# vsergeev/luaradio

Measured on AMD Instinct MI355X. Metric: MSamples/s per block (128-tap complex FIR headline) + WBFM chain end-to-end, higher is better.
Workload: dtype f32

## Files before the change

luaradio_amd/csrc/kernels_channelizer.h:

```cpp
#pragma once
#include "common.h"
#include "kernels_fir.h"

#ifndef LRHIP_CHAN_EXP
#define LRHIP_CHAN_EXP 0
#endif

namespace lrhip {

#ifndef LRHIP_CHAN_INTERLEAVE
#define LRHIP_CHAN_INTERLEAVE 1
#endif
#ifndef LRHIP_CHAN_RT
#define LRHIP_CHAN_RT 1
#endif
#ifndef LRHIP_CHAN_KSLAB
#define LRHIP_CHAN_KSLAB 32
#endif
constexpr int CHAN_RT = LRHIP_CHAN_RT;
constexpr int CHAN_MT = 64 * CHAN_RT;
constexpr int CHAN_KSLAB = LRHIP_CHAN_KSLAB;

template <int NCT>
__global__ __launch_bounds__(256, CHAN_RT == 1 ? 2 : 1) void channelizer_kernel(const float *__restrict__ hist, const float *__restrict__ x,
                                                             const float *__restrict__ W, float *__restrict__ y,
                                                             int M, long n, long nframes, long first)
{
    constexpr int K2 = 16 * NCT;
    constexpr int K = K2 / 2;
    constexpr int DROW = K2 + 2;
    constexpr int WROW = K2 + 16;
    extern __shared__ __attribute__((aligned(16))) float lds[];
    const int tid = threadIdx.x, lane = tid & 63, wave = tid >> 6;
    const int col = lane & 15, kq = lane >> 4;
    const long f0 = (long)blockIdx.x * CHAN_MT;
    const int nsamp = (CHAN_MT - 1) * K + M;
    const int nflt = 2 * nsamp;
    float *ldsD = lds;
    const int dsize = ((nflt + 2 * (nflt / K2) + 2 + 3) / 4) * 4;
    float *ldsW = lds + dsize;

    const long p0 = first + f0 * K;
    const long xlo = p0 - (M - 1);
    if (xlo >= 0 && xlo + nsamp <= n && ((reinterpret_cast<uintptr_t>(x + 2 * xlo) & 15) == 0)) {
        const float4 *src = reinterpret_cast<const float4 *>(x + 2 * xlo);
        for (int i4 = tid; i4 < nflt / 4; i4 += 256) {
            float4 v = src[i4];
            int a = 4 * i4, p = a + 2 * (a / K2);
            *reinterpret_cast<float2 *>(ldsD + p) = make_float2(v.x, v.y);
            *reinterpret_cast<float2 *>(ldsD + p + 2) = make_float2(v.z, v.w);
        }
        for (int a = (nflt / 4) * 4 + tid; a < nflt; a += 256) ldsD[a + 2 * (a / K2)] = x[2 * xlo + a];
    } else {
        for (int r = tid; r < nsamp; r += 256) {
            int a = 2 * r, p = a + 2 * (a / K2);
            ldsD[p] = stream_at<2>(hist, x, p0 + r, 0, M, n);
            ldsD[p + 1] = stream_at<2>(hist, x, p0 + r, 1, M, n);
        }
    }

    constexpr int SLAB_F4 = CHAN_KSLAB * K2 / 4;
    constexpr int UW = (SLAB_F4 + 255) / 256;
    const float4 *W4 = reinterpret_cast<const float4 *>(W);
    static_assert(UW <= 8, "W slab prefetch: at most 8 float4 per thread");
    float4 w0, w1, w2, w3, w4, w5, w6, w7;
#define LR_CHAN_FOR8(OP) OP(0) OP(1) OP(2) OP(3) OP(4) OP(5) OP(6) OP(7)
#define LR_CHAN_LOAD(U)                                                                          \
    if (U < UW) {                                                                                \
        int i4 = tid + U * 256;                                                                  \
        w##U = W4[wbase + (i4 < SLAB_F4 ? i4 : SLAB_F4 - 1)];                                    \
    }
#define LR_CHAN_PUT(U)                                                                           \
    if (U < UW) {                                                                                \
        int i4 = tid + U * 256;                                                                  \
        if (i4 < SLAB_F4) *reinterpret_cast<float4 *>(wdst + ((4 * i4) / K2) * WROW + (4 * i4) % K2) = w##U; \
    }
    {
        const size_t wbase = 0;
        float *wdst = ldsW;
        LR_CHAN_FOR8(LR_CHAN_LOAD)
        LR_CHAN_FOR8(LR_CHAN_PUT)
    }
    __syncthreads();

    f32x4 acc[CHAN_RT][NCT];
#pragma unroll
    for (int r = 0; r < CHAN_RT; r++)
#pragma unroll
        for (int c = 0; c < NCT; c++) acc[r][c] = (f32x4){0.f, 0.f, 0.f, 0.f};
    const float *abase = ldsD + DROW * (wave * 16 * CHAN_RT + col) + kq;
    const int nslabs = 2 * M / CHAN_KSLAB;
    for (int s = 0; s < nslabs; s++) {
        const float *wcur = ldsW + (s & 1) * (CHAN_KSLAB * WROW);
#if LRHIP_CHAN_EXP == 1
        const bool more = false;
#else
        const bool more = s + 1 < nslabs;
#endif
        if (more) {
            const size_t wbase = (size_t)(s + 1) * SLAB_F4;
            LR_CHAN_FOR8(LR_CHAN_LOAD)
        }
        const float *ap = abase + CHAN_KSLAB * s + 2 * ((CHAN_KSLAB * s) / K2);
        const float *bp = wcur + kq * WROW + col;
        constexpr int NST = CHAN_KSLAB / 4;
        float av[2][CHAN_RT], bv[2][NCT];
        auto fetch = [&](int buf, int st) {
#pragma unroll
            for (int r = 0; r < CHAN_RT; r++) av[buf][r] = ap[16 * r * DROW + 4 * st];
#pragma unroll
            for (int c = 0; c < NCT; c++) bv[buf][c] = bp[4 * st * WROW + 16 * c];
        };
        fetch(0, 0);
#pragma unroll
        for (int st = 0; st < NST; st++) {
#if LRHIP_CHAN_INTERLEAVE
            if (st + 1 < NST) fetch((st + 1) & 1, st + 1);
#pragma unroll
            for (int c = 0; c < NCT; c++)
#pragma unroll
                for (int r = 0; r < CHAN_RT; r++)
                    acc[r][c] = __builtin_amdgcn_mfma_f32_16x16x4f32(av[st & 1][r], bv[st & 1][c], acc[r][c], 0, 0, 0);
#pragma unroll
            for (int i = 0; i < NCT * CHAN_RT; i++) {
                __builtin_amdgcn_sched_group_barrier(0x008, 1, 0);
                __builtin_amdgcn_sched_group_barrier(0x100, 1, 0);
            }
            __builtin_amdgcn_sched_barrier(0);
#else
            if (st + 1 < NST) fetch((st + 1) & 1, st + 1);
            __builtin_amdgcn_sched_barrier(0);
#pragma unroll
            for (int c = 0; c < NCT; c++)
#pragma unroll
                for (int r = 0; r < CHAN_RT; r++)
                    acc[r][c] = __builtin_amdgcn_mfma_f32_16x16x4f32(av[st & 1][r], bv[st & 1][c], acc[r][c], 0, 0, 0);
            __builtin_amdgcn_sched_barrier(0);
#endif
        }
        if (more) {
            float *wdst = ldsW + ((s + 1) & 1) * (CHAN_KSLAB * WROW);
            LR_CHAN_FOR8(LR_CHAN_PUT)
        }
#if LRHIP_CHAN_EXP != 1
        __syncthreads();
#endif
    }

#pragma unroll
    for (int rt = 0; rt < CHAN_RT; rt++)
#pragma unroll
        for (int c = 0; c < NCT; c++)
#pragma unroll
            for (int r = 0; r < 4; r++) {
                long f = f0 + (wave * CHAN_RT + rt) * 16 + 4 * kq + r;
                if (f < nframes) y[f * K2 + 16 * c + col] = acc[rt][c][r];
            }
}

#undef LR_CHAN_FOR8
#undef LR_CHAN_LOAD
#undef LR_CHAN_PUT

}
```

luaradio_amd/csrc/lrhip.hip:

```cpp
#include "../../include/lrhip.h"

#include <cmath>
#include <map>
#include <memory>
#include <string>

#include "common.h"
#include "kernels_elem.h"
#include "kernels_fft.h"
#include "kernels_fir.h"
#include "kernels_firfft.h"
#include "kernels_firdecfft.h"
#include "kernels_firdecim.h"
#include "kernels_channelizer.h"
#include "kernels_pfb.h"
#include "kernels_iir.h"
#include "kernels_agc.h"
#include "kernels_firwin.h"
#include "kernels_firwin2.h"
#include "kernels_firfft4k.h"
#include "kernels_firpols.h"
#include "kernels_firfft64.h"
#include "kernels_interp.h"
#include "kernels_rx.h"
// ... 139 lines not shown
    q->S = input_complex ? 2 : 1;
    q->in_size = q->out_size = 4 * q->S;
    q->nb = (int)nb; q->na = (int)na; q->P = (int)na - 1;
    q->seq.nb = (int)nb; q->seq.na = (int)na;
    for (unsigned i = 0; i < nb; i++) q->seq.b[i] = b[i];
    for (unsigned i = 0; i < na; i++) q->seq.a[i] = a[i];
    q->scan = q->P >= 1 && q->P <= IIR_MAX_P && nb <= IIR_MAX_NB;
    if (q->scan) {
        int P = q->P;
        IirCoeffs &co = q->co;
        memset(&co, 0, sizeof(co));
        co.nb = (int)nb; co.P = P;
        for (unsigned i = 0; i < nb; i++) co.b[i] = (float)((double)b[i] / (double)a[0]);
        for (int i = 0; i < P; i++) co.a[i] = (float)((double)a[i + 1] / (double)a[0]);
        std::vector<double> A((size_t)P * P, 0.0), T;
        for (int k = 0; k < P; k++) A[k] = -(double)co.a[k];
        for (int r = 1; r < P; r++) A[r * P + r - 1] = 1.0;
        T = A;
        for (int s = 1; s < IIR_LC; s <<= 1) matmul(T, T, T, P);
        std::vector<float> tpow((size_t)9 * P * P);
        std::vector<double> tpow64((size_t)9 * P * P);
        const double p16 = P == 1 ? T[0] : 0.0;
        for (int k = 0; k <= 8; k++) {
            for (int i = 0; i < P * P; i++) { tpow[(size_t)k * P * P + i] = (float)T[i]; tpow64[(size_t)k * P * P + i] = T[i]; }
            if (k == 8) q->Ttile = T;
            matmul(T, T, T, P);
        }
        if (P == 1 && std::fabs(p16) < 1.0 && p16 != 0.0) {
            const int wc = (int)std::ceil(std::log(1e-12) / std::log(std::fabs(p16)));
            if (wc >= 1 && wc <= 128) q->warm_chunks = wc;
        } else if (P == 1 && p16 == 0.0) {
            q->warm_chunks = 1;
        }
        if (P >= 2 && P <= 4) {
            std::vector<double> A16(tpow64.begin(), tpow64.begin() + P * P), M = A16;
            for (int wc = 1; wc <= 128 && !q->warm_chunks; wc++) {
                double mx = 0.0;
                for (double v : M) mx = std::fabs(v) > mx ? std::fabs(v) : mx;
                if (std::isfinite(mx) && mx < 1e-12) q->warm_chunks = wc;
                matmul(M, A16, M, P);
            }
        }
        if (P == 1) {
            double acc = 1.0;
            for (int l = 0; l < 64; l++) { acc *= p16; tpow.push_back((float)acc); }
        } else if (P <= 4) {
            std::vector<double> A16(tpow64.begin(), tpow64.begin() + P * P), M = A16;
            for (int l = 0; l < 64; l++) {
                for (int i = 0; i < P * P; i++) tpow.push_back((float)M[i]);
                matmul(M, A16, M, P);
            }
        }
        if (P > 4 ? upload(q->d_tpow, tpow64.data(), tpow64.size() * sizeof(double)) : upload(q->d_tpow, tpow.data(), tpow.size() * sizeof(float))) return nullptr;
        if (upload(q->d_ttile, q->Ttile.data(), q->Ttile.size() * sizeof(double))) return nullptr;
        static const bool force_3pass = getenv("LRHIP_IIR_3PASS") != nullptr;
        std::vector<double> W = q->Ttile;
        for (int w = 1; w <= 4 && !force_3pass && !q->warm_tiles; w *= 2) {
            double mx = 0.0;
            bool finite = true;
            for (double v : W) { finite = finite && std::isfinite(v); mx = std::fabs(v) > mx ? std::fabs(v) : mx; }
            if (finite && mx < 1e-46) q->warm_tiles = w;
            matmul(W, W, W, P);
        }
    }
    if (q->reset()) return nullptr;
    return q.release();
}

lrhip_stage_t *lrhip_psd_create(unsigned n, const float *window, double scale, int logarithmic, int input_complex, int fftshift)
{
    if (!(scale > 0.0)) { set_error("psd: scale must be positive"); return nullptr; }
    FftStage *q = fft_build(n);
    if (!q) return nullptr;
    q->in_real = !input_complex;
    q->in_size = input_complex ? 8 : 4;
    q->out_size = 4;
    q->out_kind = logarithmic ? FFT_OUT_PSD_LOG : FFT_OUT_PSD;
    q->out_scale = (float)(1.0 / scale);
    q->shift = fftshift != 0;
    if (window) {
        if (upload(q->window, window, n * sizeof(float))) { delete q; return nullptr; }
        q->has_window = true;
    }
    return q;
}

lrhip_stage_t *lrhip_welch_create(unsigned n, const float *window, double scale, int logarithmic, int input_complex, unsigned overlap)
{
    if (overlap >= n) { set_error("welch: overlap %u must be smaller than the frame length %u", overlap, n); return nullptr; }
    std::unique_ptr<FftStage> psd((FftStage *)lrhip_psd_create(n, window, scale, logarithmic, input_complex, 1));
    if (!psd) return nullptr;
    std::unique_ptr<WelchStage> q(new (std::nothrow) WelchStage());
    if (!q) { set_error("out of memory"); return nullptr; }
    q->N = (int)n; q->hop = (int)(n - overlap);
    q->in_size = input_complex ? 8 : 4; q->out_size = 4;
    q->psd = std::move(psd);
    if (q->reset()) return nullptr;
    return q.release();
}

long lrhip_welch_read(lrhip_stage_t *q, float *avg_host, int reset)
{
    WelchStage *w = q ? dynamic_cast<WelchStage *>(q) : nullptr;
    if (!w) return set_error("welch_read: not a welch stage");
    long frames = w->count;
    if (frames > 0) {
        if (!avg_host) return set_error("null output buffer");
        size_t bytes = (size_t)w->N * sizeof(float);
        if (w->h_avg.reserve(bytes)) return -1;
        LR_HIP(hipMemcpyAsync(w->h_avg.p, w->sum.p, bytes, hipMemcpyDeviceToHost, ctx().stream));
        LR_HIP(hipStreamSynchronize(ctx().stream));
        const float *src = (const float *)w->h_avg.p;
        for (int i = 0; i < w->N; i++) avg_host[i] = src[i] / (float)frames;
    }
    if (reset && w->clear()) return -1;
    return frames;
}

lrhip_stage_t *lrhip_dft_create(unsigned n, int inverse, int real_side)
{
    FftStage *q = fft_build(n);
    if (!q) return nullptr;
    q->inverse = inverse != 0;
    if (!inverse) {
        q->in_real = real_side != 0;
        q->in_size = real_side ? 4 : 8;
        q->out_size = 8;
        q->out_kind = FFT_OUT_COMPLEX;
        q->out_scale = 1.0f;
    } else {
        q->in_real = 0;
        q->in_size = 8;
        q->out_size = real_side ? 4 : 8;
        q->out_kind = real_side ? FFT_OUT_REAL : FFT_OUT_COMPLEX;
        q->out_scale = (float)(1.0 / (double)n);
    }
    return q;
}

lrhip_stage_t *lrhip_format_convert_create(const char *format, int complex_out)
{
    if (!format) { set_error("format: missing format name"); return nullptr; }
    int idx = -1;
    for (size_t i = 0; i < sizeof(kFormats) / sizeof(kFormats[0]); i++)
        if (!strcmp(kFormats[i].name, format)) idx = (int)i;
    if (idx < 0) { set_error("Unsupported format (\"%s\")", format); return nullptr; }
    if (ensure_init()) return nullptr;
    FormatStage *q = new (std::nothrow) FormatStage();
    if (!q) { set_error("out of memory"); return nullptr; }
    q->fmt = idx;
    q->scalars = complex_out ? 2 : 1;
    q->in_size = kFormats[idx].bytes * q->scalars;
    q->out_size = 4 * q->scalars;
    return q;
}

lrhip_stage_t *lrhip_format_pack_create(const char *format, int complex_in)
{
    FormatStage *q = (FormatStage *)lrhip_format_convert_create(format, complex_in);
    if (!q) return nullptr;
    q->pack = true;
    std::swap(q->in_size, q->out_size);
    return q;
}

lrhip_stage_t *lrhip_multiply_constant_create(float re, float im, int constant_complex, int input_complex)
{
    if (constant_complex && !input_complex) { set_error("multiplyconstant: a complex constant takes ComplexFloat32 input only (multiplyconstant.lua:42-44)"); return nullptr; }
    if (ensure_init()) return nullptr;
    MulConstStage *q = new (std::nothrow) MulConstStage();
    if (!q) { set_error("out of memory"); return nullptr; }
    q->cr = re; q->ci = constant_complex ? im : 0.f;
    q->mode = !input_complex ? 0 : (constant_complex ? 2 : 1);
    q->in_size = q->out_size = input_complex ? 8 : 4;
    return q;
}

lrhip_stage_t *lrhip_upsampler_create(unsigned factor, int elem_size)
{
    if (factor < 1) { set_error("upsampler: factor must be >= 1"); return nullptr; }
    if (elem_size != 4 && elem_size != 8) { set_error("upsampler: element size must be 4 or 8"); return nullptr; }
    if (ensure_init()) return nullptr;
    UpsamplerStage *q = new (std::nothrow) UpsamplerStage();
    if (!q) { set_error("out of memory"); return nullptr; }
    q->factor = factor;
    q->in_size = q->out_size = elem_size;
    return q;
}

lrhip_stage_t *lrhip_agc_create(double power_alpha, double gain_alpha, double target, double threshold, int input_complex)
{
    if (!(power_alpha > 0.0 && power_alpha <= 1.0) || !(gain_alpha > 0.0 && gain_alpha <= 1.0)) { set_error("agc: alphas must be in (0, 1]"); return nullptr; }
    if (!(target > 0.0) || !(threshold >= 0.0)) { set_error("agc: target and threshold are linear powers (> 0)"); return nullptr; }
    if (ensure_init()) return nullptr;
    std::unique_ptr<AgcStage> q(new (std::nothrow) AgcStage());
    if (!q) { set_error("out of memory"); return nullptr; }
    q->p = AgcParams{power_alpha, gain_alpha, target, threshold};
    q->S = input_complex ? 2 : 1;
    q->in_size = q->out_size = 4 * q->S;
    if (q->reset()) return nullptr;
    return q.release();
}

lrhip_stage_t *lrhip_powersquelch_create(double alpha, double threshold, int input_complex)
{
    if (!(alpha > 0.0 && alpha <= 1.0)) { set_error("powersquelch: alpha must be in (0, 1]"); return nullptr; }
    AgcStage *q = (AgcStage *)lrhip_agc_create(alpha, 1.0, 1.0, threshold, input_complex);
    if (q) q->squelch = true;
    return q;
}

lrhip_stage_t *lrhip_fmmod_create(double modulation_index)
{
    if (!std::isfinite(modulation_index)) { set_error("fmmod: modulation index must be finite"); return nullptr; }
    if (ensure_init()) return nullptr;
    std::unique_ptr<FmModStage> q(new (std::nothrow) FmModStage());
    if (!q) { set_error("out of memory"); return nullptr; }
    q->k = modulation_index;
    q->in_size = 4; q->out_size = 8;
    if (q->reset()) return nullptr;
    return q.release();
}

lrhip_stage_t *lrhip_unary_create(const char *op, float re, float im, int constant_complex, int input_complex)
{
    if (!op) { set_error("unary: missing operation name"); return nullptr; }
    {
        std::string name;
        std::map<std::string, double> kv;
        const char *c = strchr(op, ':');
        const std::string head(op, c ? (size_t)(c - op) : strlen(op));
        if (head == "preamblesampler") return preamblesampler_create(op);
        if (head == "pam" || head == "qam") return modulator_create(op);
        if (head == "pll") return pll_create(op);
        if (head == "rdsframer") return plain_create<RfStage>(op, 8);
        if (head == "scmframer") return plain_create<EfStage<EF_SCM>>(op, EfProto<EF_SCM>::REC);
        if (head == "scmplusframer") return plain_create<EfStage<EF_SCMPLUS>>(op, EfProto<EF_SCMPLUS>::REC);
        if (head == "idmframer") return plain_create<EfStage<EF_IDM>>(op, EfProto<EF_IDM>::REC);
        if (head == "ax25framer") return plain_create<AxStage>(op, AX_REC);
        if (head == "pocsagframer") return plain_create<PgStage>(op, PG_REC);
        if (head == "varicodedecoder") return plain_create<VcStage>(op, 1);
        if (head == "manchesterdecoder") {
            if (!parse_op(op, name, kv, {"invert"})) return nullptr;
            return manchesterdecoder_create(kv, op);
        }
        if (c || digital_unary_op(head)) {
            if (!digital_unary_op(head)) { set_error("unary: unknown operation \"%s\"", op); return nullptr; }
            if (!parse_op(op, name, kv, digital_keys(head))) return nullptr;
            return digital_unary_create(name, kv, op);
        }
    }
    struct { const char *name; int code, in, out; } T[] = {
        {"complexmagnitude", UN_CMAG, 8, 4}, {"complexphase", UN_CPHASE, 8, 4}, {"complextoreal", UN_CREAL, 8, 4},
        {"complextoimag", UN_CIMAG, 8, 4},   {"complexconjugate", UN_CCONJ, 8, 8}, {"realtocomplex", UN_R2C, 4, 8},
        {"absolutevalue", UN_ABS, 4, 4}};
    int code = -1, in = 0, out = 0;
    for (auto &t : T)
        if (!strcmp(t.name, op)) { code = t.code; in = t.in; out = t.out; }
    if (!strcmp(op, "addconstant")) {
        if (constant_complex && !input_complex) { set_error("addconstant: a complex constant takes ComplexFloat32 input only (addconstant.lua:42-44)"); return nullptr; }
        code = !input_complex ? UN_ADDC_REAL : (constant_complex ? UN_ADDC_CPLX : UN_ADDC_CPLX_BY_REAL);
        in = out = input_complex ? 8 : 4;
    }
    if (code < 0) { set_error("unary: unknown operation \"%s\"", op); return nullptr; }
    if (ensure_init()) return nullptr;
    UnaryStage *q = new (std::nothrow) UnaryStage();
    if (!q) { set_error("out of memory"); return nullptr; }
    q->op = code; q->cr = re; q->ci = im;
    q->in_size = in; q->out_size = out;
    return q;
}

lrhip_stage_t *lrhip_delay_create(unsigned num_samples, int elem_size)
{
    if (num_samples < 1) { set_error("Number of samples must be greater than 0"); return nullptr; }
    if (elem_size != 4 && elem_size != 8) { set_error("delay: element size must be 4 or 8"); return nullptr; }
    if (ensure_init()) return nullptr;
    std::unique_ptr<DelayStage> q(new (std::nothrow) DelayStage());
    if (!q) { set_error("out of memory"); return nullptr; }
    q->D = num_samples;
    q->in_size = q->out_size = elem_size;
    if (q->reset()) return nullptr;
    return q.release();
}

lrhip_stage_t *lrhip_hilbert_create(const float *taps, unsigned ntaps)
{
    if (!taps || (ntaps % 2) != 1) { set_error("Number of taps must be odd"); return nullptr; }
    std::unique_ptr<HilbertStage> q(new (std::nothrow) HilbertStage());
    if (!q) { set_error("out of memory"); return nullptr; }
    q->fir.reset(fir_build(taps, ntaps, 0, 0, 1, 0, false, 0.0));
    if (!q->fir) return nullptr;
    q->in_size = 4; q->out_size = 8;
    return q.release();
}

lrhip_stage_t *lrhip_channelizer_create(const float *taps, unsigned ntaps, unsigned nchannels)
{
    if (!taps || ntaps < 32 || (ntaps % 32) != 0 || ntaps > 8192) { set_error("channelizer: ntaps must be a multiple of 32 in [32, 8192]"); return nullptr; }
    if (nchannels != 32 && nchannels != 64) { set_error("channelizer: nchannels must be 32 or 64"); return nullptr; }
    if (ensure_init()) return nullptr;
    std::unique_ptr<ChannelizerStage> q(new (std::nothrow) ChannelizerStage());
    if (!q) { set_error("out of memory"); return nullptr; }
    int M = (int)ntaps, K = (int)nchannels, K2 = 2 * K;
    q->M = M; q->K = K;
    q->in_size = q->out_size = 8;
    std::vector<float> W((size_t)2 * M * K2);
    const double PI2 = 6.283185307179586476925286766559;
    for (int i = 0; i < M; i++)
        for (int c = 0; c < K; c++) {
            int j = M - 1 - i;
            double a = PI2 * (double)(((long)c * j) % K) / K, h = taps[j];
            float gr = (float)(h * std::cos(a)), gi = (float)(h * std::sin(a));
            W[(size_t)(2 * i) * K2 + 2 * c] = gr;
            W[(size_t)(2 * i + 1) * K2 + 2 * c] = -gi;
            W[(size_t)(2 * i) * K2 + 2 * c + 1] = gi;
            W[(size_t)(2 * i + 1) * K2 + 2 * c + 1] = gr;
        }
    if (upload(q->W, W.data(), W.size() * sizeof(float))) return nullptr;
    if (q->reset()) return nullptr;
    return q.release();
}

lrhip_stage_t *lrhip_pfb_channelizer_create(const float *taps, unsigned ntaps, unsigned nchannels)
{
    return lrhip_pfb_oversampled_create(taps, ntaps, nchannels, 1);
}

lrhip_stage_t *lrhip_pfb_oversampled_create(const float *taps, unsigned ntaps, unsigned nchannels, unsigned oversample)
{
    if (const char *why = PfbChannelizerStage::refusal(taps ? ntaps : 0, nchannels, oversample)) { set_error("%s", why); return nullptr; }
    if (ensure_init()) return nullptr;
    std::unique_ptr<PfbChannelizerStage> q(new (std::nothrow) PfbChannelizerStage());
    if (!q) { set_error("out of memory"); return nullptr; }
    const int M = (int)ntaps, K = (int)nchannels;
    q->M = M; q->K = K; q->P = (M + K - 1) / K;
    q->R = (int)oversample; q->D = K / q->R;
    while ((1 << q->log2k) < K) q->log2k++;
    q->in_size = q->out_size = 8;
    std::vector<float> tw((size_t)K);
    for (int m = 0; m < K / 2; m++) {
        double ang = -2.0 * 3.14159265358979323846 * m / K;
        tw[2 * m] = (float)std::cos(ang);
        tw[2 * m + 1] = (float)std::sin(ang);
    }
    if (upload(q->taps, taps, (size_t)M * sizeof(float)) || upload(q->tw, tw.data(), tw.size() * sizeof(float))) return nullptr;
    if (q->reset()) return nullptr;
    return q.release();
}

lrhip_stage_t *lrhip_binary_create(const char *op, int input_complex)
{
    if (!op) { set_error("binary: missing operation name"); return nullptr; }
    if (!strcmp(op, "sampler")) {
        if (ensure_init()) return nullptr;
        std::unique_ptr<SamplerStage> q(new (std::nothrow) SamplerStage());
        if (!q) { set_error("out of memory"); return nullptr; }
        q->in_size = q->out_size = input_complex ? 8 : 4;
        q->in2_size = 4;
        if (q->reset()) return nullptr;
        return q.release();
    }
    int code = !strcmp(op, "multiply") ? BIN_MULTIPLY : !strcmp(op, "multiplyconjugate") ? BIN_MULTIPLY_CONJ
             : !strcmp(op, "add") ? BIN_ADD : !strcmp(op, "subtract") ? BIN_SUBTRACT : !strcmp(op, "floattocomplex") ? BIN_F2C : -1;
    if (code < 0) { set_error("binary: unknown operation \"%s\"", op); return nullptr; }
    if (code == BIN_MULTIPLY_CONJ && !input_complex) { set_error("binary: multiplyconjugate takes ComplexFloat32 inputs (multiplyconjugate.lua:26)"); return nullptr; }
    if (ensure_init()) return nullptr;
    BinaryStage *q = new (std::nothrow) BinaryStage();
    if (!q) { set_error("out of memory"); return nullptr; }
    q->op = code;
    q->in_size = q->out_size = input_complex ? 8 : 4;
    if (code == BIN_F2C) { q->in_size = 4; q->out_size = 8; }
    return q;
}

void lrhip_stage_destroy(lrhip_stage_t *q)
{
    if (!q) return;
    if (ctx().ready) (void)hipStreamSynchronize(ctx().stream);
    delete q;
}

int lrhip_stage_reset(lrhip_stage_t *q) { return q ? q->reset() : set_error("null stage"); }
int lrhip_stage_input_size(const lrhip_stage_t *q) { return q ? q->in_size : set_error("null stage"); }
int lrhip_stage_output_size(const lrhip_stage_t *q) { return q ? q->out_size : set_error("null stage"); }
unsigned long lrhip_stage_max_output(const lrhip_stage_t *q, unsigned long n_in) { return q ? q->max_output(n_in) : 0; }

long lrhip_stage_execute_device(lrhip_stage_t *q, const void *in_dev, unsigned long n_in, void *out_dev, unsigned long out_capacity)
{
    if (!q) return set_error("null stage");
    if (n_in && (!in_dev || (!out_dev && q->max_output(n_in)))) return set_error("null buffer");
    return q->run(in_dev, n_in, out_dev, out_capacity);
}

long lrhip_stage_execute(lrhip_stage_t *q, const void *in_host, unsigned long n_in, void *out_host, unsigned long out_capacity)
{
    if (!q) return set_error("null stage");
    return host_execute(q->h_in, q->h_out, q->d_in, q->d_out, q->in_size, q->out_size, q->max_output(n_in), in_host, n_in,
                        out_host, out_capacity,
                        [&](const void *di, unsigned long n, void *dout, unsigned long cap) { return q->run(di, n, dout, cap); }, q->align(), q->direct_io_ok());
}

long lrhip_stage_execute2_device(lrhip_stage_t *q, const void *in1_dev, const void *in2_dev, unsigned long n_in, void *out_dev,
                                 unsigned long out_capacity)
{
    if (!q) return set_error("null stage");
    if (n_in && (!in1_dev || !in2_dev || !out_dev)) return set_error("null buffer");
    return q->run2(in1_dev, in2_dev, n_in, out_dev, out_capacity);
}

long lrhip_stage_execute2(lrhip_stage_t *q, const void *in1_host, const void *in2_host, unsigned long n_in, void *out_host,
                          unsigned long out_capacity)
{
    if (!q) return set_error("null stage");
    BinaryStage *b = dynamic_cast<BinaryStage *>(q);
    if (!b) return set_error("%s is not a two-input stage", q->kind());
    if (n_in && !in2_host) return set_error("null input buffer");
    const int in2_size = q->input2_size();
    size_t bytes = (size_t)n_in * in2_size;
    if (b->h_in2.reserve(bytes ? bytes : 16) || b->d_in2.reserve(bytes ? bytes : 16)) return -1;
    if (bytes) {
        memcpy(b->h_in2.p, in2_host, bytes);
        LR_HIP(hipMemcpyAsync(b->d_in2.p, b->h_in2.p, bytes, hipMemcpyHostToDevice, ctx().stream));
    }
    return host_execute(q->h_in, q->h_out, q->d_in, q->d_out, q->in_size, q->out_size, q->max_output(n_in), in1_host, n_in, out_host, out_capacity,
                        [&](const void *di, unsigned long n, void *dout, unsigned long cap) {
                            const size_t first = (size_t)((const char *)di - (const char *)q->d_in.p) / (size_t)q->in_size;
                            return q->run2(di, (const char *)b->d_in2.p + first * (size_t)in2_size, n, dout, cap);
                        });
}

lrhip_chain_t *lrhip_chain_create(lrhip_stage_t **stages, unsigned nstages) { return lrhip_chain_create_ex(stages, nstages, 0u); }

lrhip_chain_t *lrhip_chain_create_ex(lrhip_stage_t **stages, unsigned nstages, unsigned flags)
{
    if (!stages || nstages < 1) { set_error("chain: need at least one stage"); return nullptr; }
    if (flags & ~(unsigned)(LRHIP_CHAIN_EXACT_ROTATOR | LRHIP_CHAIN_NO_POLYPHASE_TAIL | LRHIP_CHAIN_NO_FUSION | LRHIP_CHAIN_NO_SINGLE_LAUNCH)) {
        set_error("chain: unknown flag bits 0x%x", flags);
        return nullptr;
    }
    for (unsigned i = 0; i < nstages; i++)
        if (!stages[i]) { set_error("chain: stage %u is null", i); return nullptr; }
    for (unsigned i = 0; i + 1 < nstages; i++)
        if (stages[i]->out_size != stages[i + 1]->in_size) {
            set_error("chain: stage %u (%s) emits %d-byte samples but stage %u (%s) takes %d-byte samples", i, stages[i]->kind(),
                      stages[i]->out_size, i + 1, stages[i + 1]->kind(), stages[i + 1]->in_size);
            return nullptr;
        }
    std::unique_ptr<lrhip_chain> c(new (std::nothrow) lrhip_chain());
    if (!c) { set_error("out of memory"); return nullptr; }
    c->flags = flags;
    const PlanFlags pf{!(flags & LRHIP_CHAIN_NO_FUSION), (flags & LRHIP_CHAIN_EXACT_ROTATOR) != 0, (flags & LRHIP_CHAIN_NO_POLYPHASE_TAIL) != 0,
                       !(flags & LRHIP_CHAIN_NO_SINGLE_LAUNCH)};
    std::vector<lrhip_stage_t *> kept;
    if (pf.fusion && nstages > 1) {
        for (unsigned k = 0; k < nstages; k++) {
            DownsamplerStage *d1 = dynamic_cast<DownsamplerStage *>(stages[k]);
            if (!(d1 && d1->factor == 1)) kept.push_back(stages[k]);
        }
        if (!kept.empty() && kept.size() < nstages) { stages = kept.data(); nstages = (unsigned)kept.size(); }
    }
    Plan plan{stages, nstages, pf, c->ops};
    for (unsigned i = 0; i < nstages;) {
        int used = 0;
        for (size_t r = 0; pf.fusion && !used && r < sizeof kPlanRules / sizeof kPlanRules[0]; r++) used = kPlanRules[r](plan, i);
        if (used < 0) return nullptr;
        if (!used) { c->ops.emplace_back(stages[i]); used = 1; }
        i += (unsigned)used;
    }
    if (pf.fusion) {
        fold_fixups(c->ops);
        if (merge_receivers(c->ops, pf)) return nullptr;
        fold_tuner_records(c->ops);
        if (digital_fuse_tail(c->ops)) return nullptr;
    }
    for (size_t k = 0; k + 1 < c->ops.size(); k++) c->edges.emplace_back(new DeviceBuf());
    return c.release();
}

void lrhip_chain_destroy(lrhip_chain_t *c)
{
    if (!c) return;
    if (ctx().ready) (void)hipStreamSynchronize(ctx().stream);
    delete c;
}

int lrhip_chain_reset(lrhip_chain_t *c)
{
    if (!c) return set_error("null chain");
    if (c->inflight) return set_error("chain reset: %u chunks still in flight", c->inflight);
    c->fill = 0;
    c->discard_in = 0;
    if (ctx().ready) LR_HIP(hipStreamSynchronize(ctx().stream));
    for (auto &o : c->ops)
        if (o.stage->reset()) return -1;
    return 0;
}

unsigned long lrhip_chain_max_output(const lrhip_chain_t *c, unsigned long n_in)
{
    if (!c) return 0;
    unsigned long n = n_in;
    for (auto &o : c->ops) n = o.stage->max_output(n);
    return n;
}

static unsigned long chain_output_bound(const lrhip_chain *c, unsigned long n);

long lrhip_chain_execute_device(lrhip_chain_t *c, const void *in_dev, unsigned long n_in, void *out_dev, unsigned long out_capacity)
{
    if (!c) return set_error("null chain");
    g_launches = 0;
    if (c->discard_in && n_in) {
        const unsigned long k = c->discard_in < n_in ? (unsigned long)c->discard_in : n_in;
        const unsigned long bound = chain_output_bound(c, k);
        if (c->d_discard.reserve((size_t)bound * c->ops.back().stage->out_size + 16)) return -1;
        c->discard_in -= k;
        const unsigned long long left = c->discard_in;
        c->discard_in = 0;
        long rc = lrhip_chain_execute_device(c, in_dev, k, c->d_discard.p, bound);
        c->discard_in = left;
        if (rc < 0) return rc;
        in_dev = (const char *)in_dev + (size_t)k * c->ops.front().stage->in_size;
        n_in -= k;
        if (!n_in) return 0;
    }
    const void *cur = in_dev;
    unsigned long n = n_in;
    for (size_t k = 0; k < c->ops.size(); k++) {
        lrhip_stage *s = c->ops[k].stage;
        bool last = k + 1 == c->ops.size();
        unsigned long need = s->max_output(n);
        void *dst;
        unsigned long cap;
        if (last) {
            dst = out_dev;
            cap = out_capacity;
        } else {
            if (c->edges[k]->reserve((size_t)need * s->out_size + 16)) return -1;
            dst = c->edges[k]->p;
            cap = need;
        }
        long got = s->run(cur, n, dst, cap);
        if (got < 0) return got;
        cur = dst;
        n = (unsigned long)got;
    }
    c->last_launches = g_launches;
    return (long)n;
}

long lrhip_chain_execute(lrhip_chain_t *c, const void *in_host, unsigned long n_in, void *out_host, unsigned long out_capacity)
{
    if (!c) return set_error("null chain");
    return host_execute(c->h_in, c->h_out, c->d_in, c->d_out, c->ops.front().stage->in_size, c->ops.back().stage->out_size,
                        lrhip_chain_max_output(c, n_in), in_host, n_in, out_host, out_capacity,
                        [&](const void *di, unsigned long n, void *dout, unsigned long cap) { return lrhip_chain_execute_device(c, di, n, dout, cap); },
                        lrhip_chain_shard_align(c), c->ops.front().stage->direct_io_ok() && c->ops.back().stage->direct_io_ok());
}

int lrhip_chain_last_launches(const lrhip_chain_t *c) { return c ? c->last_launches : set_error("null chain"); }

int lrhip_chain_in_flight(const lrhip_chain_t *c) { return c ? (int)c->inflight : set_error("null chain"); }

static unsigned long stage_output_bound(const lrhip_stage *s, unsigned long n)
{
    unsigned long m = s->max_output(n);
    if (const FirStage *f = dynamic_cast<const FirStage *>(s))
        if (f->use_fft) m = n + (unsigned long)f->L;
    return (m > n ? m : n) + 64;
}
static unsigned long chain_output_bound(const lrhip_chain *c, unsigned long n)
{
    for (auto &o : c->ops) n = stage_output_bound(o.stage, n);
    return n;
}

int lrhip_chain_set_ring(lrhip_chain_t *c, unsigned depth, unsigned long max_chunk)
{
    if (!c) return set_error("null chain");
    if (depth < 1 || depth > 16) return set_error("ring depth must be 1..16");
    if (max_chunk < 1) return set_error("ring: max_chunk must be >= 1");
    if (c->inflight) return set_error("ring: %u chunks still in flight", c->inflight);
    if (ensure_init()) return -1;
    if (!c->s_in) LR_HIP(hipStreamCreateWithFlags(&c->s_in, hipStreamNonBlocking));
    if (!c->s_out) LR_HIP(hipStreamCreateWithFlags(&c->s_out, hipStreamNonBlocking));
    LR_HIP(hipStreamSynchronize(ctx().stream));
    c->ring.clear();
    int in_size = c->ops.front().stage->in_size, out_size = c->ops.back().stage->out_size;
    unsigned long max_out = chain_output_bound(c, max_chunk);
    for (unsigned i = 0; i < depth; i++) {
        std::unique_ptr<lrhip_chain::Slot> sl(new (std::nothrow) lrhip_chain::Slot());
        if (!sl) return set_error("out of memory");
        if (sl->h_in.reserve((size_t)max_chunk * in_size) || sl->d_in.reserve((size_t)max_chunk * in_size)) return -1;
        if (sl->h_out.reserve((size_t)max_out * out_size) || sl->d_out.reserve((size_t)max_out * out_size)) return -1;
        LR_HIP(hipEventCreateWithFlags(&sl->ev_in, hipEventDisableTiming));
        LR_HIP(hipEventCreateWithFlags(&sl->ev_done, hipEventDisableTiming));
        LR_HIP(hipEventCreateWithFlags(&sl->ev_out, hipEventDisableTiming));
        c->ring.push_back(std::move(sl));
    }
    unsigned long nmax = max_chunk;
    for (size_t k = 0; k + 1 < c->ops.size(); k++) {
        nmax = stage_output_bound(c->ops[k].stage, nmax);
        if (c->edges[k]->reserve((size_t)nmax * c->ops[k].stage->out_size + 16)) return -1;
    }
    c->ring_chunk = max_chunk;
    c->ring_out_cap = max_out;
    c->fill = 0;
    c->head = 0;
    c->inflight = 0;
    return 0;
}

static long chain_submit(lrhip_chain_t *c, const void *in_host, unsigned long n_in, bool allow_inplace);
long lrhip_chain_submit(lrhip_chain_t *c, const void *in_host, unsigned long n_in) { return chain_submit(c, in_host, n_in, true); }
static long chain_submit(lrhip_chain_t *c, const void *in_host, unsigned long n_in, bool allow_inplace)
{
    if (!c) return set_error("null chain");
    if (c->ring.empty()) return set_error("chain has no ring: call lrhip_chain_set_ring first");
    if (n_in > c->ring_chunk) return set_error("chunk of %lu samples exceeds the ring's max_chunk %lu", n_in, c->ring_chunk);
    if (c->inflight == c->ring.size()) return set_error("ring full: collect a chunk first (%u in flight)", c->inflight);
// ... 550 lines not shown
```

luaradio_amd/csrc/stage_resample.h:

```cpp
#pragma once

struct ResampleStage : lrhip_stage {
    int S = 2, M = 0, L = 1, HQ = 0;
    unsigned long D = 1;
    float c = 1.f;
    DeviceBuf d_taps, d_ttab, hist[2];
    int cur = 0;
    uint64_t Q0 = 0, m0 = 0;
    int interp_J = 0;
    int rat_blocks_per_cu = 0;
    static bool rational_supported(int L, unsigned long D) { return (L == 3 && D == 2) || (L == 2 && D == 3) || (L == 4 && D == 3) || (L == 3 && D == 4) || (L == 5 && D == 4) || (L == 4 && D == 5); }
    int interp_blocks_per_cu = 0;
    static int resample_rounds(long ntiles, long slots)
    {
        static const char *e = getenv("LRHIP_RESAMPLE_ROUNDS");
        if (e) return atoi(e) < 0 ? 0 : atoi(e);
        return ntiles <= slots ? 0 : 1;
    }
    static constexpr int SPAN_MAX = 6144;
    const char *kind() const override { return "resample"; }
    unsigned long max_output(unsigned long n) const override { return (n * (unsigned long)L) / D + 2; }
    int seek(unsigned long long n0, unsigned long long *n0_out) override
    {
        if (reset()) return -1;
        Q0 = n0;
        m0 = (n0 * (uint64_t)L + D - 1) / D;
        *n0_out = m0;
        return 0;
    }
    long memory() const override { return HQ; }
    void rate(unsigned long *num, unsigned long *den) const override { *num = D; *den = (unsigned long)L; }
    static bool fits(int M, int L, unsigned long D) { return L >= 1 && 256 * D / (unsigned long)L + (unsigned long)((M - 1) / L) + 4 <= (unsigned long)SPAN_MAX; }
    int reset() override
    {
        cur = 0; Q0 = 0; m0 = 0;
        size_t hb = (size_t)(HQ > 0 ? HQ : 1) * S * sizeof(float);
        return (zero_fill(hist[0], hb) || zero_fill(hist[1], hb)) ? -1 : 0;
    }
    long run(const void *in_dev, unsigned long n, void *out_dev, unsigned long cap) override
    {
        if (!n) return 0;
        uint64_t hi = (Q0 + n) * (uint64_t)L;
        uint64_t m_end = (hi + D - 1) / D;
        long n_out = (long)(m_end - m0);
        if ((unsigned long)n_out > cap) return set_error("resample: output capacity %lu < %ld", cap, n_out);
        const float *h = (const float *)hist[cur].p;
        float *ho = (float *)hist[cur ^ 1].p;
        if (interp_J > 0 && D == 1 && ((uintptr_t)in_dev & 7) == 0 && ((uintptr_t)out_dev & 7) == 0) {
            auto gi = [&](auto kern, size_t lds_bytes, int tq) -> int {
                if (lds_bytes > 48 * 1024) LR_HIP(hipFuncSetAttribute((const void *)kern, hipFuncAttributeMaxDynamicSharedMemorySize, (int)lds_bytes));
                if (!interp_blocks_per_cu) {
                    int nb = 0;
                    LR_HIP(hipOccupancyMaxActiveBlocksPerMultiprocessor(&nb, kern, FIP_NT, lds_bytes));
                    interp_blocks_per_cu = nb < 1 ? 1 : nb;
                }
                const long ntiles = ((long)n + tq - 1) / tq, slots = (long)ctx().num_cus * interp_blocks_per_cu;
                const int rounds = resample_rounds(ntiles, slots);
                const long wgs = rounds > 0 ? (ntiles + rounds - 1) / rounds : (ntiles < slots ? ntiles : slots);
                hipLaunchKernelGGL(kern, dim3((unsigned)wgs), dim3(FIP_NT), lds_bytes, ctx().stream, h, (const float *)in_dev, (const float *)d_ttab.p,
                                   (float *)out_dev, (long)n, HQ, c, ho, ablation_bits("LRHIP_INTERP_DBG"), rounds);
                return 0;
            };
#define LR_INTERP(LL, JJ) gi(fir_interp_kernel<LL, JJ>, (size_t)FipGeom<LL, JJ>::LDS_FLOATS * sizeof(float), FipGeom<LL, JJ>::TQ)
            int rc = L == 2 ? LR_INTERP(2, 64) : L == 3 ? LR_INTERP(3, 43) : L == 4 ? LR_INTERP(4, 32) : LR_INTERP(5, 26);
#undef LR_INTERP
            if (rc) return rc;
            LR_LAUNCH_CHECK();
            cur ^= 1;
            Q0 += n;
            m0 = m_end;
            return n_out;
        }
        static const bool no_rational = getenv("LRHIP_NO_RATIONAL_WIN") != nullptr;
        if (!no_rational && interp_J > 0 && D > 1 && ((uintptr_t)in_dev & 7) == 0 && ((uintptr_t)out_dev & 7) == 0) {
            auto gr = [&](auto kern, size_t lds_bytes, int tq) -> int {
                if (lds_bytes > 48 * 1024) LR_HIP(hipFuncSetAttribute((const void *)kern, hipFuncAttributeMaxDynamicSharedMemorySize, (int)lds_bytes));
                if (!rat_blocks_per_cu) {
                    int nb = 0;
                    LR_HIP(hipOccupancyMaxActiveBlocksPerMultiprocessor(&nb, kern, 256, lds_bytes));
                    rat_blocks_per_cu = nb < 1 ? 1 : nb;
                }
                const long ntiles = ((long)n + (long)(Q0 % D) + tq - 1) / tq, slots = (long)ctx().num_cus * rat_blocks_per_cu;
                const int rounds = resample_rounds(ntiles, slots);
                const long wgs = rounds > 0 ? (ntiles + rounds - 1) / rounds : (ntiles < slots ? ntiles : slots);
                hipLaunchKernelGGL(kern, dim3((unsigned)wgs), dim3(256), lds_bytes, ctx().stream, h, (const float *)in_dev, (const float *)d_ttab.p,
                                   (float *)out_dev, (long)n, n_out, m0, Q0, HQ, c, ho, rounds);
                return 0;
            };
#define LR_RAT(LL, DD, JJ, RR) gr(fir_rational_kernel<LL, DD, JJ, RR>, (size_t)FrrGeom<LL, DD, JJ, RR>::LDS_FLOATS * sizeof(float), FrrGeom<LL, DD, JJ, RR>::TQ)
            int rc = (L == 3 && D == 2) ? LR_RAT(3, 2, 43, 6) : (L == 2 && D == 3) ? LR_RAT(2, 3, 64, 9) : (L == 4 && D == 3) ? LR_RAT(4, 3, 32, 6)
                   : (L == 3 && D == 4) ? LR_RAT(3, 4, 43, 8) : (L == 5 && D == 4) ? LR_RAT(5, 4, 26, 8) : LR_RAT(4, 5, 32, 10);
#undef LR_RAT
            if (rc) return rc;
            LR_LAUNCH_CHECK();
            cur ^= 1;
            Q0 += n;
            m0 = m_end;
            return n_out;
        }
        int span_cap = (int)(256 * D / (unsigned long)L) + (M - 1) / L + 4;
        size_t lds_bytes = ((size_t)((((M - 1) / L + 1) * L + 3) & ~3) + (size_t)span_cap * S) * sizeof(float);
        auto go = [&](auto kern) -> int {
            if (lds_bytes > 48 * 1024) LR_HIP(hipFuncSetAttribute((const void *)kern, hipFuncAttributeMaxDynamicSharedMemorySize, (int)lds_bytes));
            unsigned grid = n_out > 0 ? (unsigned)((n_out + 255) / 256) : 1;
            hipLaunchKernelGGL(kern, dim3(grid), dim3(256), lds_bytes, ctx().stream, h, (const float *)in_dev, (const float *)d_taps.p, (float *)out_dev, M, L,
                               (long)D, (long)n, n_out, m0, Q0, HQ, c, span_cap, ho);
            return 0;
        };
        int rc = S == 2 ? go(fir_resample_kernel<2>) : go(fir_resample_kernel<1>);
        if (rc) return rc;
        LR_LAUNCH_CHECK();
        cur ^= 1;
        Q0 += n;
        m0 = m_end;
        return n_out;
    }
};

struct ChannelizerStage : lrhip_stage {
    int seek(unsigned long long, unsigned long long *) override { return set_error("seek: not supported by the channelizer stage"); }
    long memory() const override { return -1; }
    int M = 0, K = 0;
    DeviceBuf W, hist[2];
    int cur = 0;
    unsigned long index = 0;
    const char *kind() const override { return "channelizer"; }
    unsigned long max_output(unsigned long n) const override { return (n / K + 1) * K; }
    int reset() override
    {
        cur = 0; index = 0;
        size_t hb = (size_t)(M - 1) * 2 * sizeof(float);
        return (zero_fill(hist[0], hb) || zero_fill(hist[1], hb)) ? -1 : 0;
    }
    template <int NCT>
    int launch(const float *x, long n, float *y, long nframes)
    {
        constexpr int K2 = 16 * NCT;
        int nflt = 2 * ((CHAN_MT - 1) * K + M);
        size_t dsize = (size_t)((nflt + 2 * (nflt / K2) + 2 + 3) / 4) * 4;
        size_t lds_bytes = (dsize + (size_t)2 * CHAN_KSLAB * (K2 + 16)) * sizeof(float);
        auto kern = channelizer_kernel<NCT>;
        if (lds_bytes > 48 * 1024) LR_HIP(hipFuncSetAttribute((const void *)kern, hipFuncAttributeMaxDynamicSharedMemorySize, (int)lds_bytes));
        unsigned grid = (unsigned)((nframes + CHAN_MT - 1) / CHAN_MT);
        hipLaunchKernelGGL(kern, dim3(grid), dim3(256), lds_bytes, ctx().stream, (const float *)hist[cur].p, x, (const float *)W.p, y, M, n,
                           nframes, (long)index);
        LR_LAUNCH_CHECK();
        return 0;
    }
    long run(const void *in_dev, unsigned long n_in, void *out_dev, unsigned long cap) override
    {
        long n = (long)n_in;
        if (n <= 0) return 0;
        long nframes = n_in > index ? (long)((n_in - index + K - 1) / K) : 0;
        if ((unsigned long)(nframes * K) > cap) return set_error("channelizer: output capacity %lu < %ld", cap, nframes * K);
        const float *x = (const float *)in_dev;
        if (nframes > 0) {
            int rc = K == 32 ? launch<4>(x, n, (float *)out_dev, nframes) : launch<8>(x, n, (float *)out_dev, nframes);
            if (rc) return rc;
        }
        unsigned grid = grid_for((unsigned long)(M - 1) * 2, 256);
        hipLaunchKernelGGL(fir_history_kernel<2>, dim3(grid), dim3(256), 0, ctx().stream, (const float *)hist[cur].p, x, (float *)hist[cur ^ 1].p, M, n);
        LR_LAUNCH_CHECK();
        cur ^= 1;
        index = index + (unsigned long)nframes * K - n_in;
        return nframes * K;
    }
};
```

Before: 328,200.

## Restructure channelizer GEMM with real cos/sin table and planar real/imag input

Replaces the complex-interleaved 2M x 2K weight matrix with a real M x K table holding cosine and sine columns for half the channels. The input is split into separate real and imaginary LDS planes, and mirrored channel outputs are reconstructed from pairs of real products. This removes redundant multiplications by exploiting conjugate symmetry of the DFT twiddles for real taps, roughly quartering the weight table and halving the MFMA work. In exchange it adds a combining epilogue with scattered float2 stores, and it only supports K of 32 or 64.

```diff
diff --git a/luaradio_amd/csrc/channelizer_table.h b/luaradio_amd/csrc/channelizer_table.h
--- /dev/null
+++ b/luaradio_amd/csrc/channelizer_table.h
@@ -0,0 +1,50 @@
+#pragma once
+#include <cmath>
+#include <cstddef>
+#include <vector>
+
+#if defined(__HIPCC__)
+#define LR_CHAN_HD __host__ __device__ inline
+#else
+#define LR_CHAN_HD inline
+#endif
+
+namespace lrhip {
+
+struct ChanColumn { int channel; bool sine; };
+
+inline ChanColumn chan_column(int j, int K)
+{
+    if (j <= K / 2) return {j, false};
+    return {j - K / 2, true};
+}
+
+inline int chan_cos_column(int k) { return k; }
+inline int chan_sin_column(int k, int K) { return K / 2 + k; }
+
+inline std::vector<float> chan_paired_table(const float *taps, int M, int K)
+{
+    std::vector<float> W((size_t)M * K);
+    const double PI2 = 6.283185307179586476925286766559;
+    for (int i = 0; i < M; i++)
+        for (int j = 0; j < K; j++) {
+            const ChanColumn col = chan_column(j, K);
+            const int t = M - 1 - i;
+            const double a = PI2 * (double)(((long)col.channel * t) % K) / K, h = taps[t];
+            W[(size_t)i * K + j] = (float)(h * (col.sine ? std::sin(a) : std::cos(a)));
+        }
+    return W;
+}
+
+struct ChanOut { float re, im; };
+LR_CHAN_HD void chan_pair_outputs(float prc, float pic, float prs, float pis, ChanOut &yk, ChanOut &ymirror)
+{
+    yk.re = prc - pis;      yk.im = prs + pic;
+    ymirror.re = prc + pis; ymirror.im = pic - prs;
+}
+LR_CHAN_HD ChanOut chan_self_output(float prc, float pic)
+{
+    return {prc + 0.0f * pic, pic + 0.0f * prc};
+}
+
+}
diff --git a/luaradio_amd/csrc/kernels_channelizer.h b/luaradio_amd/csrc/kernels_channelizer.h
--- a/luaradio_amd/csrc/kernels_channelizer.h
+++ b/luaradio_amd/csrc/kernels_channelizer.h
@@ -1,70 +1,71 @@
 #pragma once
 #include "common.h"
 #include "kernels_fir.h"
-
-#ifndef LRHIP_CHAN_EXP
-#define LRHIP_CHAN_EXP 0
-#endif
+#include "channelizer_table.h"
 
 namespace lrhip {
 
-#ifndef LRHIP_CHAN_INTERLEAVE
-#define LRHIP_CHAN_INTERLEAVE 1
-#endif
-#ifndef LRHIP_CHAN_RT
-#define LRHIP_CHAN_RT 1
-#endif
 #ifndef LRHIP_CHAN_KSLAB
 #define LRHIP_CHAN_KSLAB 32
 #endif
-constexpr int CHAN_RT = LRHIP_CHAN_RT;
-constexpr int CHAN_MT = 64 * CHAN_RT;
+#ifndef LRHIP_CHAN_WGS
+#define LRHIP_CHAN_WGS 2
+#endif
+constexpr int CHAN_WGS = LRHIP_CHAN_WGS;
+constexpr int CHAN_MT = 64;
 constexpr int CHAN_KSLAB = LRHIP_CHAN_KSLAB;
+static_assert(32 % CHAN_KSLAB == 0 && CHAN_KSLAB % 4 == 0, "a W' slab must divide every accepted tap count (multiples of 32) and hold whole k-steps");
+
+__host__ __device__ constexpr int chan_plane_floats(int nsamp, int K) { return ((nsamp + 2 * (nsamp / K) + 2 + 3) / 4) * 4; }
 
 template <int NCT>
-__global__ __launch_bounds__(256, CHAN_RT == 1 ? 2 : 1) void channelizer_kernel(const float *__restrict__ hist, const float *__restrict__ x,
+__global__ __launch_bounds__(256, CHAN_WGS) void channelizer_kernel(const float *__restrict__ hist, const float *__restrict__ x,
                                                              const float *__restrict__ W, float *__restrict__ y,
                                                              int M, long n, long nframes, long first)
 {
-    constexpr int K2 = 16 * NCT;
-    constexpr int K = K2 / 2;
-    constexpr int DROW = K2 + 2;
-    constexpr int WROW = K2 + 16;
+    constexpr int K = 16 * NCT;
+    constexpr int HCT = NCT / 2;
+    constexpr int PROW = K + 2;
+    constexpr int WROW = K + 16;
+    static_assert(K % CHAN_KSLAB == 0, "a slab must not straddle a padded plane row");
     extern __shared__ __attribute__((aligned(16))) float lds[];
     const int tid = threadIdx.x, lane = tid & 63, wave = tid >> 6;
     const int col = lane & 15, kq = lane >> 4;
     const long f0 = (long)blockIdx.x * CHAN_MT;
     const int nsamp = (CHAN_MT - 1) * K + M;
-    const int nflt = 2 * nsamp;
-    float *ldsD = lds;
-    const int dsize = ((nflt + 2 * (nflt / K2) + 2 + 3) / 4) * 4;
-    float *ldsW = lds + dsize;
+    const int psize = chan_plane_floats(nsamp, K);
+    float *ldsR = lds, *ldsI = lds + psize;
+    float *ldsW = lds + 2 * psize;
 
     const long p0 = first + f0 * K;
     const long xlo = p0 - (M - 1);
     if (xlo >= 0 && xlo + nsamp <= n && ((reinterpret_cast<uintptr_t>(x + 2 * xlo) & 15) == 0)) {
         const float4 *src = reinterpret_cast<const float4 *>(x + 2 * xlo);
-        for (int i4 = tid; i4 < nflt / 4; i4 += 256) {
+        for (int i4 = tid; i4 < nsamp / 2; i4 += 256) {
             float4 v = src[i4];
-            int a = 4 * i4, p = a + 2 * (a / K2);
-            *reinterpret_cast<float2 *>(ldsD + p) = make_float2(v.x, v.y);
-            *reinterpret_cast<float2 *>(ldsD + p + 2) = make_float2(v.z, v.w);
+            int r = 2 * i4, p = r + 2 * (r / K);
+            *reinterpret_cast<float2 *>(ldsR + p) = make_float2(v.x, v.z);
+            *reinterpret_cast<float2 *>(ldsI + p) = make_float2(v.y, v.w);
         }
-        for (int a = (nflt / 4) * 4 + tid; a < nflt; a += 256) ldsD[a + 2 * (a / K2)] = x[2 * xlo + a];
+        for (int r = (nsamp / 2) * 2 + tid; r < nsamp; r += 256) {
+            int p = r + 2 * (r / K);
+            ldsR[p] = x[2 * (xlo + r)];
+            ldsI[p] = x[2 * (xlo + r) + 1];
+        }
     } else {
         for (int r = tid; r < nsamp; r += 256) {
-            int a = 2 * r, p = a + 2 * (a / K2);
-            ldsD[p] = stream_at<2>(hist, x, p0 + r, 0, M, n);
-            ldsD[p + 1] = stream_at<2>(hist, x, p0 + r, 1, M, n);
+            int p = r + 2 * (r / K);
+            ldsR[p] = stream_at<2>(hist, x, p0 + r, 0, M, n);
+            ldsI[p] = stream_at<2>(hist, x, p0 + r, 1, M, n);
         }
     }
 
-    constexpr int SLAB_F4 = CHAN_KSLAB * K2 / 4;
+    constexpr int SLAB_F4 = CHAN_KSLAB * K / 4;
     constexpr int UW = (SLAB_F4 + 255) / 256;
     const float4 *W4 = reinterpret_cast<const float4 *>(W);
-    static_assert(UW <= 8, "W slab prefetch: at most 8 float4 per thread");
-    float4 w0, w1, w2, w3, w4, w5, w6, w7;
-#define LR_CHAN_FOR8(OP) OP(0) OP(1) OP(2) OP(3) OP(4) OP(5) OP(6) OP(7)
+    static_assert(UW <= 2, "W' slab prefetch: at most 2 float4 per thread");
+    float4 w0, w1;
+#define LR_CHAN_FOR2(OP) OP(0) OP(1)
 #define LR_CHAN_LOAD(U)                                                                          \
     if (U < UW) {                                                                                \
         int i4 = tid + U * 256;                                                                  \
@@ -73,92 +74,90 @@
 #define LR_CHAN_PUT(U)                                                                           \
     if (U < UW) {                                                                                \
         int i4 = tid + U * 256;                                                                  \
-        if (i4 < SLAB_F4) *reinterpret_cast<float4 *>(wdst + ((4 * i4) / K2) * WROW + (4 * i4) % K2) = w##U; \
+        if (i4 < SLAB_F4) *reinterpret_cast<float4 *>(wdst + ((4 * i4) / K) * WROW + (4 * i4) % K) = w##U; \
     }
     {
         const size_t wbase = 0;
         float *wdst = ldsW;
-        LR_CHAN_FOR8(LR_CHAN_LOAD)
-        LR_CHAN_FOR8(LR_CHAN_PUT)
+        LR_CHAN_FOR2(LR_CHAN_LOAD)
+        LR_CHAN_FOR2(LR_CHAN_PUT)
     }
     __syncthreads();
 
-    f32x4 acc[CHAN_RT][NCT];
+    f32x4 acc[2][NCT];
 #pragma unroll
-    for (int r = 0; r < CHAN_RT; r++)
+    for (int r = 0; r < 2; r++)
 #pragma unroll
         for (int c = 0; c < NCT; c++) acc[r][c] = (f32x4){0.f, 0.f, 0.f, 0.f};
-    const float *abase = ldsD + DROW * (wave * 16 * CHAN_RT + col) + kq;
-    const int nslabs = 2 * M / CHAN_KSLAB;
+    const int aoff = PROW * (wave * 16 + col) + kq;
+    const int nslabs = M / CHAN_KSLAB;
     for (int s = 0; s < nslabs; s++) {
         const float *wcur = ldsW + (s & 1) * (CHAN_KSLAB * WROW);
-#if LRHIP_CHAN_EXP == 1
-        const bool more = false;
-#else
         const bool more = s + 1 < nslabs;
-#endif
         if (more) {
             const size_t wbase = (size_t)(s + 1) * SLAB_F4;
-            LR_CHAN_FOR8(LR_CHAN_LOAD)
+            LR_CHAN_FOR2(LR_CHAN_LOAD)
         }
-        const float *ap = abase + CHAN_KSLAB * s + 2 * ((CHAN_KSLAB * s) / K2);
+        const int soff = aoff + CHAN_KSLAB * s + 2 * ((CHAN_KSLAB * s) / K);
+        const float *apr = ldsR + soff, *api = ldsI + soff;
         const float *bp = wcur + kq * WROW + col;
         constexpr int NST = CHAN_KSLAB / 4;
-        float av[2][CHAN_RT], bv[2][NCT];
+        float av[2][2], bv[2][NCT];
         auto fetch = [&](int buf, int st) {
-#pragma unroll
-            for (int r = 0; r < CHAN_RT; r++) av[buf][r] = ap[16 * r * DROW + 4 * st];
+            av[buf][0] = apr[4 * st];
+            av[buf][1] = api[4 * st];
 #pragma unroll
             for (int c = 0; c < NCT; c++) bv[buf][c] = bp[4 * st * WROW + 16 * c];
         };
         fetch(0, 0);
 #pragma unroll
         for (int st = 0; st < NST; st++) {
-#if LRHIP_CHAN_INTERLEAVE
             if (st + 1 < NST) fetch((st + 1) & 1, st + 1);
 #pragma unroll
             for (int c = 0; c < NCT; c++)
 #pragma unroll
-                for (int r = 0; r < CHAN_RT; r++)
+                for (int r = 0; r < 2; r++)
                     acc[r][c] = __builtin_amdgcn_mfma_f32_16x16x4f32(av[st & 1][r], bv[st & 1][c], acc[r][c], 0, 0, 0);
 #pragma unroll
-            for (int i = 0; i < NCT * CHAN_RT; i++) {
+            for (int i = 0; i < 2 * NCT; i++) {
                 __builtin_amdgcn_sched_group_barrier(0x008, 1, 0);
                 __builtin_amdgcn_sched_group_barrier(0x100, 1, 0);
             }
             __builtin_amdgcn_sched_barrier(0);
-#else
-            if (st + 1 < NST) fetch((st + 1) & 1, st + 1);
-            __builtin_amdgcn_sched_barrier(0);
-#pragma unroll
-            for (int c = 0; c < NCT; c++)
-#pragma unroll
-                for (int r = 0; r < CHAN_RT; r++)
-                    acc[r][c] = __builtin_amdgcn_mfma_f32_16x16x4f32(av[st & 1][r], bv[st & 1][c], acc[r][c], 0, 0, 0);
-            __builtin_amdgcn_sched_barrier(0);
-#endif
         }
         if (more) {
             float *wdst = ldsW + ((s + 1) & 1) * (CHAN_KSLAB * WROW);
-            LR_CHAN_FOR8(LR_CHAN_PUT)
+            LR_CHAN_FOR2(LR_CHAN_PUT)
         }
-#if LRHIP_CHAN_EXP != 1
         __syncthreads();
-#endif
     }
 
+    float2 *y2 = reinterpret_cast<float2 *>(y);
 #pragma unroll
-    for (int rt = 0; rt < CHAN_RT; rt++)
+    for (int t = 0; t < HCT; t++)
 #pragma unroll
-        for (int c = 0; c < NCT; c++)
-#pragma unroll
-            for (int r = 0; r < 4; r++) {
-                long f = f0 + (wave * CHAN_RT + rt) * 16 + 4 * kq + r;
-                if (f < nframes) y[f * K2 + 16 * c + col] = acc[rt][c][r];
+        for (int r = 0; r < 4; r++) {
+            const long f = f0 + wave * 16 + 4 * kq + r;
+            const int k = 16 * t + col;
+            const float prc = acc[0][t][r], pic = acc[1][t][r], prs = acc[0][t + HCT][r], pis = acc[1][t + HCT][r];
+            ChanOut a, b;
+            int kb;
+            if (k == 0) {
+                a = chan_self_output(prc, pic);
+                b = chan_self_output(prs, pis);
+                kb = K / 2;
+            } else {
+                chan_pair_outputs(prc, pic, prs, pis, a, b);
+                kb = K - k;
             }
+            if (f < nframes) {
+                y2[f * K + k] = make_float2(a.re, a.im);
+                y2[f * K + kb] = make_float2(b.re, b.im);
+            }
+        }
 }
 
-#undef LR_CHAN_FOR8
+#undef LR_CHAN_FOR2
 #undef LR_CHAN_LOAD
 #undef LR_CHAN_PUT
 
diff --git a/luaradio_amd/csrc/lrhip.hip b/luaradio_amd/csrc/lrhip.hip
--- a/luaradio_amd/csrc/lrhip.hip
+++ b/luaradio_amd/csrc/lrhip.hip
@@ -465,21 +465,10 @@
     if (ensure_init()) return nullptr;
     std::unique_ptr<ChannelizerStage> q(new (std::nothrow) ChannelizerStage());
     if (!q) { set_error("out of memory"); return nullptr; }
-    int M = (int)ntaps, K = (int)nchannels, K2 = 2 * K;
+    int M = (int)ntaps, K = (int)nchannels;
     q->M = M; q->K = K;
     q->in_size = q->out_size = 8;
-    std::vector<float> W((size_t)2 * M * K2);
-    const double PI2 = 6.283185307179586476925286766559;
-    for (int i = 0; i < M; i++)
-        for (int c = 0; c < K; c++) {
-            int j = M - 1 - i;
-            double a = PI2 * (double)(((long)c * j) % K) / K, h = taps[j];
-            float gr = (float)(h * std::cos(a)), gi = (float)(h * std::sin(a));
-            W[(size_t)(2 * i) * K2 + 2 * c] = gr;
-            W[(size_t)(2 * i + 1) * K2 + 2 * c] = -gi;
-            W[(size_t)(2 * i) * K2 + 2 * c + 1] = gi;
-            W[(size_t)(2 * i + 1) * K2 + 2 * c + 1] = gr;
-        }
+    const std::vector<float> W = chan_paired_table(taps, M, K);
     if (upload(q->W, W.data(), W.size() * sizeof(float))) return nullptr;
     if (q->reset()) return nullptr;
     return q.release();
diff --git a/luaradio_amd/csrc/stage_resample.h b/luaradio_amd/csrc/stage_resample.h
--- a/luaradio_amd/csrc/stage_resample.h
+++ b/luaradio_amd/csrc/stage_resample.h
@@ -135,10 +135,9 @@
     template <int NCT>
     int launch(const float *x, long n, float *y, long nframes)
     {
-        constexpr int K2 = 16 * NCT;
-        int nflt = 2 * ((CHAN_MT - 1) * K + M);
-        size_t dsize = (size_t)((nflt + 2 * (nflt / K2) + 2 + 3) / 4) * 4;
-        size_t lds_bytes = (dsize + (size_t)2 * CHAN_KSLAB * (K2 + 16)) * sizeof(float);
+        static_assert(NCT == 2 || NCT == 4, "K = 16 NCT in {32, 64}: an even number of column tiles, cosine and sine halves");
+        size_t lds_bytes = ((size_t)2 * chan_plane_floats((CHAN_MT - 1) * K + M, K) + (size_t)2 * CHAN_KSLAB * (K + 16)) * sizeof(float);
+        if (CHAN_WGS == 1 && lds_bytes <= 80 * 1024) lds_bytes = 80 * 1024 + 16;
         auto kern = channelizer_kernel<NCT>;
         if (lds_bytes > 48 * 1024) LR_HIP(hipFuncSetAttribute((const void *)kern, hipFuncAttributeMaxDynamicSharedMemorySize, (int)lds_bytes));
         unsigned grid = (unsigned)((nframes + CHAN_MT - 1) / CHAN_MT);
@@ -155,7 +154,7 @@
         if ((unsigned long)(nframes * K) > cap) return set_error("channelizer: output capacity %lu < %ld", cap, nframes * K);
         const float *x = (const float *)in_dev;
         if (nframes > 0) {
-            int rc = K == 32 ? launch<4>(x, n, (float *)out_dev, nframes) : launch<8>(x, n, (float *)out_dev, nframes);
+            int rc = K == 32 ? launch<2>(x, n, (float *)out_dev, nframes) : launch<4>(x, n, (float *)out_dev, nframes);
             if (rc) return rc;
         }
         unsigned grid = grid_for((unsigned long)(M - 1) * 2, 256);
```

Measured after the change: 315,500. -3.9%, worse.
